# hsp-iit/online-detection

Measured on AMD Instinct MI355X. Metric: FALKON fit+infer samples/sec (N=1e6 D=1024 M=1e4), higher is better.
Workload: dtype f32-accurate K_nM (X Z' as a two-term f16 split on the f16 MFMA, f32 accumulate) stored as 24-bit fixed point (step 2^-24) + f64 solver (preconditioner: K_MM, T and T^-1 in f64; the products of the A factor, which only preconditions, at f32 accuracy on the f16 MFMA)

## Files before the change

online-detection_amd/csrc/api.cpp:

```cpp
#include "odx_common.h"
#include <string.h>

namespace odx {
static thread_local char g_error[512] = "";

void set_error(const char* fmt, ...) {
  va_list ap;
  va_start(ap, fmt);
  vsnprintf(g_error, sizeof(g_error), fmt, ap);
  va_end(ap);
}
}

extern "C" const char* odx_last_error_string(void) { return odx::g_error; }

#include "odx_internal.h"
namespace odx {
struct OptSpec {
  const char* name;
  int def, lo, hi;
};
constexpr int T_INVERSE_UNMERGED_DEFAULT = 2;
static const OptSpec g_opt_spec[OPT_COUNT] = {
    {"h2_tile", 0, 0, 256}, {"precond", 0, 0, 2}, {"chain_helpers", -1, -1, 1}, {"rls_force_nt_gram", 0, 0, 1},
    {"rls_force_inverse_solve", 0, 0, 1}, {"t_inverse_unmerged", T_INVERSE_UNMERGED_DEFAULT, 0, 2}, {"t_inverse_force_stop", 0, 0, 1 << 20}};
static int g_opt[OPT_COUNT] = {0, 0, -1, 0, 0, T_INVERSE_UNMERGED_DEFAULT, 0};
int lib_option(int which) { return g_opt[which]; }
static int opt_index(const char* name) {
  if (name)
    for (int i = 0; i < OPT_COUNT; ++i)
      if (strcmp(name, g_opt_spec[i].name) == 0) return i;
  return -1;
}
}

extern "C" int odx_set_option(const char* name, int value) {
  const int i = odx::opt_index(name);
  ODX_REQUIRE(i >= 0, "odx_set_option: unknown option '%s'", name ? name : "(null)");
  const odx::OptSpec& sp = odx::g_opt_spec[i];
  ODX_REQUIRE(value >= sp.lo && value <= sp.hi && (i != odx::OPT_H2_TILE || value == 0 || value == 128 || value == 256),
              "odx_set_option: %s = %d out of range", name, value);
  odx::g_opt[i] = value;
  return ODX_OK;
}

extern "C" int odx_get_option(const char* name, int* value) {
  const int i = odx::opt_index(name);
  ODX_REQUIRE(i >= 0 && value, "odx_get_option: unknown option '%s'", name ? name : "(null)");
  *value = odx::g_opt[i];
  return ODX_OK;
}

extern "C" int odx_option_default(const char* name, int* value) {
  const int i = odx::opt_index(name);
  ODX_REQUIRE(i >= 0 && value, "odx_option_default: unknown option '%s'", name ? name : "(null)");
  *value = odx::g_opt_spec[i].def;
  return ODX_OK;
}

extern "C" int odx_version(void) { return 100; }

extern "C" int odx_device_cus(void) {
  int dev = 0;
  if (hipGetDevice(&dev) != hipSuccess) {
    odx::set_error("odx_device_cus: no HIP device");
    return ODX_ERR_HIP;
  }
  int cus = 0;
  if (hipDeviceGetAttribute(&cus, hipDeviceAttributeMultiprocessorCount, dev) != hipSuccess) {
    odx::set_error("odx_device_cus: attribute query failed");
    return ODX_ERR_HIP;
  }
  return cus;
// ... 38 lines not shown
```

online-detection_amd/csrc/dense_f64.hip:

```cpp
#include "odx_internal.h"
#include <vector>

namespace odx {

typedef double f64x2 __attribute__((ext_vector_type(2)));
typedef double f64x4v __attribute__((ext_vector_type(4)));

constexpr int DB_NB = POTRF_NB;
constexpr int DB_LD = DB_NB + 1;
constexpr int DB_XLD = 33;
constexpr int DB_NT = 512;
constexpr int DB_PQ = 3072 / DB_NT;

__device__ __forceinline__ double readlane_f64(double v, int src) {
  const long long b = __double_as_longlong(v);
  const unsigned lo = (unsigned)__builtin_amdgcn_readlane((int)(b & 0xffffffffll), src);
  const unsigned hi = (unsigned)__builtin_amdgcn_readlane((int)(b >> 32), src);
  return __longlong_as_double((long long)(((unsigned long long)hi << 32) | lo));
}

__device__ __forceinline__ void chol32_wave(double* s, double* rd, int J, int jb, int32_t* info, int info_base,
                                            int lane) {
  const int l = lane & 31;
  double row[32];
// ... 577 lines not shown
  ODX_CHECK_LAUNCH("add_diag_f64");
  return ODX_OK;
}

int fill_f64(double* A, int64_t lda, int64_t rows, int64_t cols, double value, hipStream_t stream) {
  if (rows <= 0 || cols <= 0) return ODX_OK;
  ODX_REQUIRE(rows < 65536 * 32768ll, "fill_f64: too many rows");
  for (int64_t r0 = 0; r0 < rows; r0 += 65535) {
    const int64_t nr = rows - r0 < 65535 ? rows - r0 : 65535;
    hipLaunchKernelGGL(fill_f64_kernel, dim3((unsigned)ceil_div(cols, 256), (unsigned)nr), dim3(256), 0, stream,
                       A + r0 * lda, lda, nr, cols, value);
  }
  ODX_CHECK_LAUNCH("fill_f64");
  return ODX_OK;
}

__global__ __launch_bounds__(DB_NT) void trtri_diag_kernel(const double* __restrict__ L, int64_t ldl, int64_t M,
                                                          double* __restrict__ Dinv, int64_t zstrideA,
                                                          int64_t zstrideD) {
  __shared__ double s[DB_NB * DB_LD];
  L += (int64_t)blockIdx.y * zstrideA;
  Dinv += (int64_t)blockIdx.y * zstrideD;
  __shared__ double xi[32 * DB_XLD];
  const int64_t r0 = (int64_t)blockIdx.x * DB_NB;
  const int jb = (int)(M - r0 < DB_NB ? M - r0 : DB_NB);
  __shared__ double rd[32];
  lds_load_lower_128(s, L + r0 * ldl + r0, ldl, jb);
  lds_trinv_128<false>(s, xi, rd, nullptr);
  lds_store_dinv_128(s, Dinv + (int64_t)blockIdx.x * DB_NB * DB_NB, jb);
}

struct SideStream {
  hipStream_t stream = nullptr;
  hipEvent_t fork = nullptr, join = nullptr;
  int device = -1;
  bool owned = true;
};

static std::vector<uint32_t> g_side_mask;
static hipStream_t g_given_helper[2] = {nullptr, nullptr};

constexpr int64_t CHAIN_HELPER_MIN_M = 4096;

static bool chain_helpers(int64_t M) {
  const int o = lib_option(OPT_CHAIN_HELPERS);
  if (o == 0 || o == 1) return o == 1;
  return M >= CHAIN_HELPER_MIN_M;
}

struct SideEntry {
  int device;
  hipStream_t caller;
  SideStream ss[2];
};
static thread_local std::vector<SideEntry*> g_side_pool;

static int release_side_streams(bool wait = true) {
  for (SideEntry* e : g_side_pool) {
    for (SideStream& s : e->ss) {
      if (s.stream != nullptr) {
        if (wait) ODX_CHECK_HIP(hipStreamSynchronize(s.stream));
        if (s.owned) ODX_CHECK_HIP(hipStreamDestroy(s.stream));
      }
      if (s.fork != nullptr) ODX_CHECK_HIP(hipEventDestroy(s.fork));
      if (s.join != nullptr) ODX_CHECK_HIP(hipEventDestroy(s.join));
    }
    delete e;
  }
  g_side_pool.clear();
  return ODX_OK;
}

static int side_stream(SideStream** out, int slot, hipStream_t caller, int64_t M) {
  typedef SideEntry Entry;
  std::vector<Entry*>& pool = g_side_pool;
  int dev = 0;
  ODX_CHECK_HIP(hipGetDevice(&dev));
  ODX_REQUIRE(slot >= 0 && slot < 2, "side_stream: bad slot");
  if (!chain_helpers(M)) {
    static thread_local SideStream inl[2];
    SideStream& s = inl[slot];
    if (s.fork == nullptr || s.device != dev) {
      ODX_CHECK_HIP(hipEventCreateWithFlags(&s.fork, hipEventDisableTiming));
      ODX_CHECK_HIP(hipEventCreateWithFlags(&s.join, hipEventDisableTiming));
      s.device = dev;
    }
    s.stream = caller;
    *out = &s;
    return ODX_OK;
  }
  Entry* e = nullptr;
  for (Entry* c : pool)
    if (c->device == dev && c->caller == caller) e = c;
  if (e == nullptr) {
    e = new Entry();
    e->device = dev;
    e->caller = caller;
    pool.push_back(e);
  }
  SideStream& s = e->ss[slot];
  if (s.stream == nullptr) {
    s.owned = true;
    if (g_given_helper[slot] != nullptr && g_side_mask.empty()) {
      s.stream = g_given_helper[slot];
      s.owned = false;
    } else if (!g_side_mask.empty()) {
      ODX_CHECK_HIP(hipExtStreamCreateWithCUMask(&s.stream, (uint32_t)g_side_mask.size(), g_side_mask.data()));
    } else if (slot == 1) {
      int lo = 0, hi = 0;
      ODX_CHECK_HIP(hipDeviceGetStreamPriorityRange(&lo, &hi));
      ODX_CHECK_HIP(hipStreamCreateWithPriority(&s.stream, hipStreamNonBlocking, lo));
    } else {
      ODX_CHECK_HIP(hipStreamCreateWithFlags(&s.stream, hipStreamNonBlocking));
    }
    ODX_CHECK_HIP(hipEventCreateWithFlags(&s.fork, hipEventDisableTiming));
    ODX_CHECK_HIP(hipEventCreateWithFlags(&s.join, hipEventDisableTiming));
    s.device = dev;
  }
  *out = &s;
  return ODX_OK;
}

constexpr int POTRF_NBO = 512;

static bool precond_split(int64_t M) {
  const int o = lib_option(OPT_PRECOND);
  if (o == 1) return false;
  if (o == 2) return true;
  return M >= 4096;
}
static int64_t precond_pack_units(int64_t M) { return 2 * M * h2_f64_packed_ld(M); }
static int64_t precond_split_doubles(int64_t M) { return (precond_pack_units(M) + 2 * M * POTRF_NBO) / 2 + 2; }
static float split_scale_for(double bound) {
  int e = 0;
  frexp(bound > 1e-300 ? bound : 1.0, &e);
  return ldexpf(1.f, 12 - e);
}


int potrf_f64(double* A, int64_t lda, int64_t M, double* Dinv, int32_t* info, hipStream_t stream, const ZBatch& zb, uint32_t* pk,
              int64_t pk_buf, int64_t pk_z, float pk_scale) {
  constexpr int NB = POTRF_NB;
  ODX_REQUIRE(lda % 2 == 0 && aligned16(A) && aligned16(Dinv), "potrf_f64: A/Dinv must be 16-byte aligned, lda even");
  const int Z = zb.count;
  ODX_REQUIRE(Z >= 1 && Z <= ODX_MAX_ZBATCH && zb.strideA % 2 == 0 && zb.strideD % 2 == 0,
              "potrf_f64: class batch of 1..%d matrices, even strides", ODX_MAX_ZBATCH);
  auto zgemm = [&](GemmParams<double>& g) {
    g.zbatches = Z; g.zstrideA = zb.strideA; g.zstrideB = zb.strideA; g.zstrideC = zb.strideA;
  };
  ODX_CHECK_HIP(hipFuncSetAttribute(reinterpret_cast<const void*>(trsm128_kernel), hipFuncAttributeMaxDynamicSharedMemorySize,
                                    TS_LDS_BYTES));
  SideStream* look = nullptr;
  ODX_PROPAGATE(side_stream(&look, 1, stream, M));
  bool pending = false;
  for (int64_t K0 = 0; K0 < M; K0 += POTRF_NBO) {
    const int64_t kbo = M - K0 < POTRF_NBO ? M - K0 : POTRF_NBO;
    for (int64_t k0 = K0; k0 < K0 + kbo; k0 += NB) {
      const int jb = (int)(M - k0 < NB ? M - k0 : NB);
      double* D = Dinv + (k0 / NB) * NB * NB;
      hipLaunchKernelGGL((potrf_diag_kernel<NB, false>), dim3((unsigned)Z), dim3(DB_NT), 0, stream, A + k0 * lda + k0, lda,
                         jb, D, info, (int)k0, zb.strideA, zb.strideD);
      ODX_CHECK_LAUNCH("potrf_diag");
      const int64_t m = M - k0 - jb;
      if (m <= 0) break;
      double* A21 = A + (k0 + jb) * lda + k0;
      hipLaunchKernelGGL(trsm128_kernel, dim3((unsigned)ceil_div(m, TS_R), (unsigned)Z), dim3(256), TS_LDS_BYTES, stream,
                         A21, lda, m, A + k0 * lda + k0, D + NB * NB - 4096, zb.strideA, zb.strideD);
      ODX_CHECK_LAUNCH("trsm128");
      const int64_t pc = (K0 + kbo) - (k0 + jb);
      if (pc > 0) {
        GemmParams<double> u;
        u.A = A21; u.lda = lda; u.B = A21; u.ldb = lda; u.C = A + (k0 + jb) * lda + (k0 + jb); u.ldc = lda;
        u.m = m; u.n = pc; u.k = jb; u.alpha = -1.0; u.beta = 1.0; u.flags = ODX_GEMM_LOWER_ONLY;
        zgemm(u);
        ODX_PROPAGATE(launch_gemm_f64(u, stream));
      }
    }
    const int64_t mt = M - K0 - kbo;
    if (mt > 0) {
      double* P = A + (K0 + kbo) * lda + K0;
      const int64_t nw = mt < POTRF_NBO ? mt : POTRF_NBO;
      if (pending) {
        ODX_CHECK_HIP(hipStreamWaitEvent(stream, look->join, 0));
        pending = false;
      }
      const int64_t mr = mt - nw;
      double minus1[ODX_MAX_ZBATCH];
      for (int z = 0; z < Z; ++z) minus1[z] = -1.0;
      uint32_t* Pk = pk ? pk + ((K0 / POTRF_NBO) & 1) * pk_buf : nullptr;
      if (Pk) {
        ODX_PROPAGATE(split_f64(P, lda, zb.strideA, mt, kbo, pk_scale, Pk, POTRF_NBO, pk_z, Z, stream));
        ODX_PROPAGATE(gemm_h2_f64(Pk, POTRF_NBO, pk_z, pk_scale, Pk, POTRF_NBO, pk_z, pk_scale, A + (K0 + kbo) * (lda + 1), lda,
                                  zb.strideA, mt, nw, kbo, minus1, 1.0, ODX_GEMM_LOWER_ONLY, Z, stream));
      } else {
        GemmParams<double> u;
        u.A = P; u.lda = lda; u.B = P; u.ldb = lda; u.C = A + (K0 + kbo) * (lda + 1); u.ldc = lda;
        u.m = mt; u.n = nw; u.k = kbo; u.alpha = -1.0; u.beta = 1.0; u.flags = ODX_GEMM_LOWER_ONLY;
        zgemm(u);
        ODX_PROPAGATE(launch_gemm_f64(u, stream));
      }
      if (mr > 0) {
        ODX_CHECK_HIP(hipEventRecord(look->fork, stream));
        ODX_CHECK_HIP(hipStreamWaitEvent(look->stream, look->fork, 0));
        if (Pk) {
          ODX_PROPAGATE(gemm_h2_f64(Pk + nw * POTRF_NBO, POTRF_NBO, pk_z, pk_scale, Pk + nw * POTRF_NBO, POTRF_NBO, pk_z, pk_scale,
                                    A + (K0 + kbo + nw) * (lda + 1), lda, zb.strideA, mr, mr, kbo, minus1, 1.0, ODX_GEMM_LOWER_ONLY, Z,
                                    look->stream));
        } else {
          double* P2 = P + nw * lda;
          GemmParams<double> r;
          r.A = P2; r.lda = lda; r.B = P2; r.ldb = lda; r.C = A + (K0 + kbo + nw) * (lda + 1); r.ldc = lda;
// ... 346 lines not shown
  SideStream* side = nullptr;
  ODX_PROPAGATE(side_stream(&side, 0, s, M));
  hipStream_t s2 = side->stream;
  const int64_t wld = precond_ld(M), ldzd = precond_ldz(D);
  const int64_t dsz = ceil_div(M, POTRF_NB) * POTRF_NB * POTRF_NB;
  double* Zd = static_cast<double*>(workspace);
  double* zsq = Zd + M * ldzd;
  double* W0 = zsq + round_up(M, 2);
  double* W1 = W0 + M * wld;
  double* W2 = W1 + M * wld;
  double* W3 = W2 + M * wld;
  double* DinvT = W3 + M * wld;
  double* DinvA = DinvT + dsz;
  const bool split = precond_split(M);
  const int64_t ldpt = h2_f64_packed_ld(M);
  uint32_t* Tk = reinterpret_cast<uint32_t*>(DinvA + dsz);
  uint32_t* Pk = Tk + precond_pack_units(M);
  double* WA = L > 1 ? static_cast<double*>(workspace) + round_up(odx_falkon_precond_workspace_bytes(M, D), 16) / (int64_t)sizeof(double) : W2;

  ODX_CHECK_HIP(hipMemsetAsync(info, 0, (size_t)L * sizeof(int32_t), s));
  ODX_CHECK_HIP(hipMemsetAsync(Zd, 0, (size_t)(M * ldzd) * sizeof(double), s));
  ODX_PROPAGATE(odx_convert_f32_f64(Z, ldz, Zd, ldzd, M, D, stream));
  ODX_CHECK_HIP(hipMemsetAsync(W0, 0, (size_t)(M * wld) * sizeof(double), s));
  ODX_PROPAGATE(gauss_kmm_f64(Zd, ldzd, M, D, sigma, eps * (double)M, W0, wld, zsq, s, kind));
  ODX_PROPAGATE(potrf_f64(W0, wld, M, DinvT, info, s));
  for (int l = 1; l < L; ++l)
    ODX_CHECK_HIP(hipMemcpyAsync(info + l, info, sizeof(int32_t), hipMemcpyDeviceToDevice, s));
  ODX_CHECK_HIP(hipEventRecord(side->fork, s));
  ODX_CHECK_HIP(hipStreamWaitEvent(s2, side->fork, 0));
  ODX_PROPAGATE(fill_f64(LTi, ld, M, M, 0.0, s2));
  ODX_PROPAGATE(fill_f64(LTit, ld, M, M, 0.0, s2));
  ODX_PROPAGATE(trtri_from_diag_f64(W0, wld, M, DinvT, LTi, LTit, ld, W3, s2));
  ODX_CHECK_HIP(hipEventRecord(side->join, s2));
  ODX_CHECK_HIP(hipMemsetAsync(W1, 0, (size_t)(M * wld) * sizeof(double), s));
  ODX_PROPAGATE(transpose_f64(W0, wld, W1, wld, M, M, s));
  ODX_CHECK_HIP(hipMemsetAsync(W2, 0, (size_t)(M * wld) * sizeof(double), s));
  if (split) {
    const float st = split_scale_for(sqrt(1.0 + eps * 65536.0));
    const double a1 = 1.0 / (double)M;
    ODX_PROPAGATE(split_f64(W1, wld, 0, M, M, st, Tk, ldpt, 0, 1, s));
    ODX_PROPAGATE(gemm_h2_f64(Tk, ldpt, 0, st, Tk, ldpt, 0, st, W2, wld, 0, M, M, M, &a1, 0.0,
                              ODX_GEMM_LOWER_ONLY | ODX_GEMM_A_UPPER | ODX_GEMM_B_UPPER, 1, s));
  } else {
    GemmParams<double> g;
    g.A = W1; g.lda = wld; g.B = W1; g.ldb = wld; g.C = W2; g.ldc = wld;
    g.m = M; g.n = M; g.k = M; g.alpha = 1.0 / (double)M; g.beta = 0.0;
    g.flags = ODX_GEMM_LOWER_ONLY | ODX_GEMM_A_UPPER | ODX_GEMM_B_UPPER;
    ODX_PROPAGATE(launch_gemm_f64(g, s));
  }
  for (int l = 0; l < L; ++l) {
    const double lam = lams[l];
    if (WA != W2) ODX_CHECK_HIP(hipMemcpyAsync(WA, W2, (size_t)(M * wld) * sizeof(double), hipMemcpyDeviceToDevice, s));
    ODX_PROPAGATE(add_diag_f64(WA, wld, M, lam, s));
    if (split) ODX_PROPAGATE(potrf_f64(WA, wld, M, DinvA, info + l, s, ZBatch(), Pk, M * POTRF_NBO, 0, split_scale_for(sqrt(1.0 + eps + lam))));
    else ODX_PROPAGATE(potrf_f64(WA, wld, M, DinvA, info + l, s));
    if (l == 0) ODX_CHECK_HIP(hipStreamWaitEvent(s, side->join, 0));
    ODX_PROPAGATE(fill_f64(LAi[l], ld, M, M, 0.0, s));
    ODX_PROPAGATE(fill_f64(LAit[l], ld, M, M, 0.0, s));
    if (split && eps + lam > 0.0)
      ODX_PROPAGATE(trtri_from_diag_f64(WA, wld, M, DinvA, LAi[l], LAit[l], ld, W1, s, ZBatch(), Tk, precond_pack_units(M), 0,
                                        sqrt(1.0 + eps + lam), 1.0 / sqrt(eps + lam)));
    else
      ODX_PROPAGATE(trtri_from_diag_f64(WA, wld, M, DinvA, LAi[l], LAit[l], ld, W1, s));
  }
  return ODX_OK;
}

extern "C" int64_t odx_falkon_precond_batched_workspace_bytes(int64_t Mmax, int D, int B) {
  if (Mmax <= 0 || D <= 0 || B <= 0) return 0;
  const int64_t ld = precond_ld(Mmax), ldzd = precond_ldz(D);
  const int64_t per = Mmax * ldzd + round_up(Mmax, 2) + 4 * Mmax * ld + 2 * ceil_div(Mmax, POTRF_NB) * POTRF_NB * POTRF_NB +
                      precond_split_doubles(Mmax);
  return per * B * (int64_t)sizeof(double);
}

static int falkon_precond_batched_f64_impl(const float* const* Z, const int64_t* ldz, const int64_t* M, int B,
                                           int64_t Mmax, int D, double sigma, double lam, double eps, int64_t t_stop, double* out,
                                           int64_t ld, int64_t out_stride, int32_t* info, void* workspace,
                                           int64_t workspace_bytes, odx_stream_t stream);

extern "C" int odx_falkon_precond_batched_f64(const float* const* Z, const int64_t* ldz, const int64_t* M, int B,
                                              int64_t Mmax, int D, double sigma, double lam, double eps, double* out,
                                              int64_t ld, int64_t out_stride, int32_t* info, void* workspace,
                                              int64_t workspace_bytes, odx_stream_t stream) {
  const int rc = falkon_precond_batched_f64_impl(Z, ldz, M, B, Mmax, D, sigma, lam, eps, 0, out, ld, out_stride, info, workspace, workspace_bytes, stream);
  return rc;
}
// ... 14 lines not shown
  ODX_REQUIRE(Z && ldz && M && out && info && workspace && Mmax > 0 && D > 0 && sigma > 0,
              "odx_falkon_precond_batched_f64: null pointer or bad size");
  ODX_REQUIRE(ld % 2 == 0 && ld >= Mmax && aligned16(out) && out_stride % 2 == 0 && out_stride >= 4 * Mmax * ld,
              "odx_falkon_precond_batched_f64: out must be 16-byte aligned, ld even >= Mmax, out_stride >= 4 Mmax ld");
  ODX_REQUIRE(aligned16(workspace), "odx_falkon_precond_batched_f64: workspace must be 16-byte aligned");
  for (int b = 0; b < B; ++b)
    ODX_REQUIRE(Z[b] && M[b] > 0 && M[b] <= Mmax, "odx_falkon_precond_batched_f64: class %d: need 0 < M <= Mmax", b);
  if (workspace_bytes < odx_falkon_precond_batched_workspace_bytes(Mmax, D, B)) {
    set_error("odx_falkon_precond_batched_f64: workspace too small");
    return ODX_ERR_WORKSPACE;
  }
  hipStream_t s = as_stream(stream);
  SideStream* side = nullptr;
  ODX_PROPAGATE(side_stream(&side, 0, s, Mmax));
  hipStream_t s2 = side->stream;
  const int64_t wld = precond_ld(Mmax), ldzd = precond_ldz(D);
  const int64_t dsz = ceil_div(Mmax, POTRF_NB) * POTRF_NB * POTRF_NB;
  const int64_t zper = Mmax * ldzd + round_up(Mmax, 2), wsz = Mmax * wld;
  double* Zd0 = static_cast<double*>(workspace);
  double* W0 = Zd0 + (int64_t)B * zper;
  double* W1 = W0 + (int64_t)B * wsz;
  double* W2 = W1 + (int64_t)B * wsz;
  double* W3 = W2 + (int64_t)B * wsz;
  double* DinvT = W3 + (int64_t)B * wsz;
  double* DinvA = DinvT + (int64_t)B * dsz;
  double* LTi = out, *LTit = out + Mmax * ld, *LAi = out + 2 * Mmax * ld, *LAit = out + 3 * Mmax * ld;
  const bool split = precond_split(Mmax);
  const int64_t ldpt = h2_f64_packed_ld(Mmax);
  uint32_t* Tk = reinterpret_cast<uint32_t*>(DinvA + (int64_t)B * dsz);
  uint32_t* Pk = Tk + (int64_t)B * precond_pack_units(Mmax);

  ODX_CHECK_HIP(hipMemsetAsync(info, 0, (size_t)B * sizeof(int32_t), s));
  ODX_CHECK_HIP(hipMemsetAsync(Zd0, 0, (size_t)((int64_t)B * zper) * sizeof(double), s));
  ODX_CHECK_HIP(hipMemsetAsync(W0, 0, (size_t)(3 * (int64_t)B * wsz) * sizeof(double), s));
  if (out_stride == 4 * Mmax * ld) {
    ODX_CHECK_HIP(hipMemsetAsync(out, 0, (size_t)((int64_t)B * out_stride) * sizeof(double), s));
  } else {
    for (int b = 0; b < B; ++b)
      ODX_CHECK_HIP(hipMemsetAsync(out + (int64_t)b * out_stride, 0, (size_t)(4 * Mmax * ld) * sizeof(double), s));
  }
  VecBatch kb;
  kb.B = B;
  for (int b = 0; b < B; ++b) {
    ODX_PROPAGATE(odx_convert_f32_f64(Z[b], ldz[b], Zd0 + (int64_t)b * zper, ldzd, M[b], D, stream));
    kb.M[b] = (int)M[b];
    kb.scale[b] = eps * (double)M[b];
  }
  ODX_PROPAGATE(gauss_kmm_f64_batched(Zd0, ldzd, zper, Mmax * ldzd, kb, D, sigma, W0, wld, wsz, s));
  for (int b = 0; b < B; ++b)
    if (M[b] < Mmax) ODX_PROPAGATE(add_diag_f64(W0 + (int64_t)b * wsz + M[b] * (wld + 1), wld, Mmax - M[b], 1.0, s));
  ZBatch zt;
  zt.count = B; zt.strideA = wsz; zt.strideD = dsz; zt.strideO = out_stride; zt.strideW = wsz;
  ODX_PROPAGATE(potrf_f64(W0, wld, Mmax, DinvT, info, s, zt));
  ODX_CHECK_HIP(hipEventRecord(side->fork, s));
  ODX_CHECK_HIP(hipStreamWaitEvent(s2, side->fork, 0));
  ODX_PROPAGATE(trtri_from_diag_f64(W0, wld, Mmax, DinvT, LTi, LTit, ld, W3, s2, zt, nullptr, 0, 0, 1.0, 1.0, t_stop));
  ODX_CHECK_HIP(hipEventRecord(side->join, s2));
  ODX_PROPAGATE(transpose_f64(W0, wld, W1, wld, Mmax, Mmax, s, B, wsz, wsz));
  if (split) {
    const float st = split_scale_for(sqrt(1.0 + eps * 65536.0)), sa = split_scale_for(sqrt(1.0 + eps + lam));
    double a1[ODX_MAX_ZBATCH];
    for (int b = 0; b < B; ++b) a1[b] = 1.0 / (double)M[b];
    ODX_PROPAGATE(split_f64(W1, wld, wsz, Mmax, Mmax, st, Tk, ldpt, precond_pack_units(Mmax), B, s));
    ODX_PROPAGATE(gemm_h2_f64(Tk, ldpt, precond_pack_units(Mmax), st, Tk, ldpt, precond_pack_units(Mmax), st, W2, wld, wsz, Mmax, Mmax, Mmax, a1, 0.0,
                              ODX_GEMM_LOWER_ONLY | ODX_GEMM_A_UPPER | ODX_GEMM_B_UPPER, B, s));
    ODX_PROPAGATE(add_diag_f64(W2, wld, Mmax, lam, s, B, wsz));
    ODX_PROPAGATE(potrf_f64(W2, wld, Mmax, DinvA, info, s, zt, Pk, (int64_t)B * Mmax * POTRF_NBO, Mmax * POTRF_NBO, sa));
  } else {
    GemmParams<double> g;
    g.A = W1; g.lda = wld; g.B = W1; g.ldb = wld; g.C = W2; g.ldc = wld;
    g.m = Mmax; g.n = Mmax; g.k = Mmax; g.beta = 0.0;
    g.flags = ODX_GEMM_LOWER_ONLY | ODX_GEMM_A_UPPER | ODX_GEMM_B_UPPER;
    g.zbatches = B; g.zstrideA = wsz; g.zstrideB = wsz; g.zstrideC = wsz;
    g.zalpha_on = 1;
    for (int b = 0; b < B; ++b) g.zalpha[b] = 1.0 / (double)M[b];
    ODX_PROPAGATE(launch_gemm_f64(g, s));
    ODX_PROPAGATE(add_diag_f64(W2, wld, Mmax, lam, s, B, wsz));
    ODX_PROPAGATE(potrf_f64(W2, wld, Mmax, DinvA, info, s, zt));
  }
  ODX_CHECK_HIP(hipStreamWaitEvent(s, side->join, 0));
  if (split && eps + lam > 0.0)
    return trtri_from_diag_f64(W2, wld, Mmax, DinvA, LAi, LAit, ld, W1, s, zt, Tk, precond_pack_units(Mmax), precond_pack_units(Mmax),
                               sqrt(1.0 + eps + lam), 1.0 / sqrt(eps + lam));
  return trtri_from_diag_f64(W2, wld, Mmax, DinvA, LAi, LAit, ld, W1, s, zt);
}

extern "C" int odx_set_side_stream_cu_mask(const uint32_t* mask, int words) {
  ODX_REQUIRE(words >= 0 && words <= 64 && (words == 0 || mask != nullptr), "odx_set_side_stream_cu_mask: bad argument");
  g_side_mask.assign(mask, mask + words);
  return ODX_OK;
}

extern "C" int odx_set_helper_streams(odx_stream_t s0, odx_stream_t s1) {
  g_given_helper[0] = reinterpret_cast<hipStream_t>(s0);
  g_given_helper[1] = reinterpret_cast<hipStream_t>(s1);
  return ODX_OK;
}

extern "C" int odx_release_helper_streams(void) {
  return odx::release_side_streams(false);
// ... 2 lines not shown
```

online-detection_amd/csrc/gauss_h2.hip:

```cpp
#include <stdlib.h>
#include <type_traits>
#include "gemm_core.h"
#include "odx_internal.h"

namespace odx {

typedef _Float16 f16x8 __attribute__((ext_vector_type(8)));

constexpr int H2_KT = 64;

__global__ __launch_bounds__(256) void absmax_f32_kernel(const float* __restrict__ X, int64_t ldx, int64_t n, int D,
                                                         unsigned int* __restrict__ out) {
  unsigned int m = 0;
  const int lane = threadIdx.x & 63;
  for (int64_t r = (int64_t)blockIdx.x * 4 + (threadIdx.x >> 6); r < n; r += (int64_t)gridDim.x * 4) {
    const float* x = X + r * ldx;
    for (int c0 = lane * 4; c0 < D; c0 += 1024) {
      u32x4 v[4];
#pragma unroll
      for (int u = 0; u < 4; ++u) {
        const int c = c0 + 256 * u;
        v[u] = (c < D) ? *reinterpret_cast<const u32x4*>(x + c) : u32x4{0u, 0u, 0u, 0u};
      }
#pragma unroll
// ... 1486 lines not shown
  *reinterpret_cast<u32x4*>(P + row * ldp + f) = v;
}

__global__ __launch_bounds__(256) void split_f64_kernel(const double* __restrict__ X, int64_t ldx, int64_t zsx, int64_t rows, int cols,
                                                        float s, uint32_t* __restrict__ P, int64_t ldp, int64_t zsp) {
  const int groups = (int)((cols + H2_KT - 1) / H2_KT) * 8;
  const int64_t row = blockIdx.y;
  const int g = blockIdx.x * 256 + threadIdx.x;
  if (g >= groups || row >= rows) return;
  const double* x = X + (int64_t)blockIdx.z * zsx + row * ldx + (int64_t)g * 8;
  double v[8];
  if (g * 8 + 8 <= cols) {
#pragma unroll
    for (int q = 0; q < 8; q += 2) {
      const f64x2 a = *reinterpret_cast<const f64x2*>(x + q);
      v[q] = a[0];
      v[q + 1] = a[1];
    }
  } else {
#pragma unroll
    for (int q = 0; q < 8; ++q) v[q] = (g * 8 + q < cols) ? x[q] : 0.0;
  }
  f16x8 hi, lo;
#pragma unroll
  for (int q = 0; q < 8; ++q) {
    const float t = (float)(v[q] * (double)s);
    const _Float16 h = (_Float16)t;
    hi[q] = h;
    lo[q] = (_Float16)(t - (float)h);
  }
  uint32_t* dst = P + (int64_t)blockIdx.z * zsp + row * ldp + (int64_t)(g >> 2) * 32 + (g & 3) * 4;
  *reinterpret_cast<f16x8*>(dst) = hi;
  *reinterpret_cast<f16x8*>(dst + 16) = lo;
}

struct H2F64Params {
  const uint32_t* PA; int64_t ldpa, zsa, bsa;
  const uint32_t* PB; int64_t ldpb, zsb, bsb;
  double* C; int64_t ldc, zsc, bsc;
  double* C2; int64_t ldc2, zsc2, bsc2;
  int64_t m, n, k;
  int64_t rg_total, rg_off, rg_step;
  int k_is_m;
  int flags;
  double beta;
  double alpha[ODX_MAX_ZBATCH];
};

struct SplitBlocks {
  const double* X; int64_t ldx, bsx, zsx;
  uint32_t* P; int64_t ldp, bsp, zsp;
  int64_t rows, cols;
  int64_t rg_total, rg_off, rg_step;
  int rows_ragged, cols_ragged, Z;
  float s;
};

__global__ __launch_bounds__(256) void split_f64_blocks_kernel(SplitBlocks p) {
  const int b = blockIdx.z / p.Z, z = blockIdx.z % p.Z;
  int64_t rg = p.rg_total - p.rg_off - (int64_t)b * p.rg_step;
  const int64_t rows = p.rows_ragged ? (rg < p.rows ? (rg > 0 ? rg : 0) : p.rows) : p.rows;
  const int64_t cols = p.cols_ragged ? (rg < p.cols ? (rg > 0 ? rg : 0) : p.cols) : p.cols;
  const int64_t row = blockIdx.y;
  const int groups = (int)((cols + H2_KT - 1) / H2_KT) * 8;
  const int g = blockIdx.x * 256 + threadIdx.x;
  if (g >= groups || row >= rows) return;
// ... 332 lines not shown

static int check_packed_pair(const char* who, int64_t dp, int64_t ldpx, int64_t ldpz, const void* PX, const void* PZ) {
  ODX_REQUIRE(ldpx % 4 == 0 && ldpz % 4 == 0 && ldpx >= dp && ldpz >= dp && aligned16(PX) && aligned16(PZ),
              "%s: packed operands must be 16-byte aligned with ld %% 4 == 0 and ld >= %lld 4-byte units", who, (long long)dp);
  ODX_REQUIRE(ldpx < (1 << 24) && ldpz < (1 << 24), "%s: leading dimensions must stay below 2^24 (32-bit tile offsets)", who);
  return ODX_OK;
}

static int check_knm_block(const char* who, int fmt, int64_t M, const void* K, int64_t ldk, const void* Klo, int64_t ldlo) {
  const int64_t ldmin = odx_knm_ld(M, fmt);
  ODX_REQUIRE(K && ldk >= ldmin && ldk % (fmt == ODX_KNM_F32 ? 4 : 8) == 0 && aligned16(K),
              "%s: K must be 16-byte aligned with ldk a multiple of %d and >= %lld", who, fmt == ODX_KNM_F32 ? 4 : 8, (long long)ldmin);
  if (fmt == ODX_KNM_U24)
    ODX_REQUIRE(Klo && ldlo >= ldmin && ldlo % 8 == 0 && aligned16(Klo), "%s: the low-byte plane must be 16-byte aligned with ldlo %% 8 == 0, ldlo >= roundup(M, 8)", who);
  ODX_REQUIRE(ldk < (1 << 24), "%s: leading dimensions must stay below 2^24 (32-bit tile offsets)", who);
  return ODX_OK;
}

int64_t h2_f64_packed_ld(int64_t cols) { return round_up(cols, H2_KT); }

int split_f64(const double* X, int64_t ldx, int64_t zsx, int64_t rows, int64_t cols, float scale, uint32_t* P, int64_t ldp,
              int64_t zsp, int z, hipStream_t stream) {
  if (rows <= 0 || cols <= 0 || z <= 0) return ODX_OK;
  ODX_REQUIRE(ldx % 2 == 0 && aligned16(X) && zsx % 2 == 0, "split_f64: X must be 16-byte aligned with even ld / class stride");
  ODX_REQUIRE(ldp % 4 == 0 && ldp >= round_up(cols, H2_KT) && aligned16(P) && zsp % 4 == 0, "split_f64: packed rows cover roundup(cols, 64)");
  ODX_REQUIRE(rows < 65536 && z < 65536, "split_f64: too many rows");
  const int groups = (int)(round_up(cols, H2_KT) / 8);
  hipLaunchKernelGGL(split_f64_kernel, dim3((unsigned)ceil_div(groups, 256), (unsigned)rows, (unsigned)z), dim3(256), 0, stream, X, ldx, zsx,
                     rows, (int)cols, scale, P, ldp, zsp);
  ODX_CHECK_LAUNCH("split_f64");
  return ODX_OK;
}

int split_f64_blocks(const SplitBlocksArgs& a, hipStream_t stream) {
  if (a.rows <= 0 || a.cols <= 0 || a.nb <= 0 || a.Z <= 0) return ODX_OK;
  ODX_REQUIRE(a.ldx % 2 == 0 && aligned16(a.X) && a.zsx % 2 == 0 && a.bsx % 2 == 0, "split_f64_blocks: X blocks must be 16-byte aligned");
  ODX_REQUIRE(a.ldp % 4 == 0 && a.ldp >= round_up(a.cols, H2_KT) && aligned16(a.P) && a.zsp % 4 == 0 && a.bsp % 4 == 0,
              "split_f64_blocks: packed rows cover roundup(cols, 64)");
  ODX_REQUIRE(a.rows < 65536 && (int64_t)a.nb * a.Z < 65536, "split_f64_blocks: too many rows / blocks");
  SplitBlocks p;
  p.X = a.X; p.ldx = a.ldx; p.bsx = a.bsx; p.zsx = a.zsx; p.P = a.P; p.ldp = a.ldp; p.bsp = a.bsp; p.zsp = a.zsp;
  p.rows = a.rows; p.cols = a.cols; p.rg_total = a.rg_total; p.rg_off = a.rg_off; p.rg_step = a.rg_step;
  p.rows_ragged = a.rows_ragged; p.cols_ragged = a.cols_ragged; p.Z = a.Z; p.s = a.scale;
  const int groups = (int)(round_up(a.cols, H2_KT) / 8);
  hipLaunchKernelGGL(split_f64_blocks_kernel, dim3((unsigned)ceil_div(groups, 256), (unsigned)a.rows, (unsigned)(a.nb * a.Z)), dim3(256), 0,
                     stream, p);
  ODX_CHECK_LAUNCH("split_f64_blocks");
  return ODX_OK;
}

int gemm_h2_f64_ex(const H2F64Args& a, hipStream_t stream) {
  if (a.m <= 0 || a.n <= 0 || a.zcount <= 0 || a.nb <= 0) return ODX_OK;
  ODX_REQUIRE(a.zcount <= ODX_MAX_ZBATCH && a.nb < 65536 && a.ldc % 2 == 0 && a.zsc % 2 == 0 && a.bsc % 2 == 0 && aligned16(a.C),
              "gemm_h2_f64: C must be 16-byte aligned, even ld / strides");
  ODX_REQUIRE(a.C2 == nullptr || (a.ldc2 % 2 == 0 && a.zsc2 % 2 == 0 && a.bsc2 % 2 == 0 && aligned16(a.C2)), "gemm_h2_f64: C2 alignment");
  ODX_REQUIRE(!(a.flags & ODX_GEMM_STORE_T) || a.beta == 0.0, "gemm_h2_f64: a transposed store cannot accumulate");
  ODX_REQUIRE(a.ldpa < (1 << 24) && a.ldpb < (1 << 24) && a.ldpa >= round_up(a.k, H2_KT) && a.ldpb >= round_up(a.k, H2_KT),
              "gemm_h2_f64: packed leading dimensions");
  H2F64Params p;
  p.PA = a.PA; p.ldpa = a.ldpa; p.zsa = a.zsa; p.bsa = a.bsa; p.PB = a.PB; p.ldpb = a.ldpb; p.zsb = a.zsb; p.bsb = a.bsb;
  p.C = a.C; p.ldc = a.ldc; p.zsc = a.zsc; p.bsc = a.bsc; p.C2 = a.C2; p.ldc2 = a.ldc2; p.zsc2 = a.zsc2; p.bsc2 = a.bsc2;
  p.m = a.m; p.n = a.n; p.k = a.k; p.rg_total = a.rg_total; p.rg_off = a.rg_off; p.rg_step = a.rg_step; p.k_is_m = a.k_is_m;
  p.flags = a.flags; p.beta = a.beta;
  for (int z = 0; z < a.zcount; ++z) p.alpha[z] = a.alpha[z] / ((double)a.sa * (double)a.sb);
  const int64_t wt = round_up(ceil_div(a.m, W_BM), 4) * ceil_div(a.n, W_BN);
  ODX_REQUIRE(wt < (1ll << 31), "gemm_h2_f64: grid too large");
// ... 1153 lines not shown
```

online-detection_amd/csrc/odx_internal.h:

```cpp
#pragma once
#include "odx_common.h"

namespace odx {
enum LibOpt {
  OPT_H2_TILE = 0,
  OPT_PRECOND,
  OPT_CHAIN_HELPERS,
  OPT_RLS_FORCE_NT_GRAM,
  OPT_RLS_FORCE_INVERSE_SOLVE,
  OPT_T_INVERSE_UNMERGED,
  OPT_T_INVERSE_FORCE_STOP,
  OPT_COUNT
};
int lib_option(int which);


constexpr int ODX_MAX_ZBATCH = 32;

template <typename T>
struct GemmParams {
  const T* A = nullptr; int64_t lda = 0;
  const T* B = nullptr; int64_t ldb = 0;
  T* C = nullptr; int64_t ldc = 0;
  T* C2 = nullptr; int64_t ldc2 = 0;
  int64_t m = 0, n = 0, k = 0;
  T alpha = T(1), beta = T(0);
  int flags = 0;
  int batches = 1;
  int64_t strideA = 0, strideB = 0, strideC = 0, strideC2 = 0;
  int64_t ragged_total = 0, ragged_off = 0, ragged_step = 0;
  int ragged_k_is_m = 0;
  int vec_epilogue = 0;
  int zbatches = 1;
  int64_t zstrideA = 0, zstrideB = 0, zstrideC = 0, zstrideC2 = 0;
  int zalpha_on = 0;
  T zalpha[ODX_MAX_ZBATCH] = {};
  int zk_on = 0;
  int64_t zkoff[ODX_MAX_ZBATCH] = {};
  int64_t zklen[ODX_MAX_ZBATCH] = {};
};

int launch_gemm_f64(const GemmParams<double>& p, hipStream_t stream);
int launch_gemm_f32(const GemmParams<float>& p, hipStream_t stream);

// ... 28 lines not shown
int knm_passq_batched(int B, const void* const* Khi, const int64_t* ldk, const void* const* Klo, const int64_t* ldlo, int fmt,
                      const int64_t* n, const int64_t* M, const double* v, int64_t vstride, double* out, int64_t ostride,
                      void* workspace, int64_t workspace_bytes, hipStream_t stream);

int pass_cus();
int check_q_block(const char* who, const void* K, int64_t ldk, const void* Klo, int64_t ldlo, int fmt, int64_t M);

bool knm_pass_batch_cfg(int B, const int64_t* M, int* nt, int* ch, int* r);
int64_t knm_pass_batched_workspace_bytes(int B, const int64_t* n, const int64_t* M);
int knm_pass_batched(int B, const float* const* K, const int64_t* ldk, const int64_t* n, const int64_t* M, const double* v,
                     int64_t vstride, double* out, int64_t ostride, void* workspace, int64_t workspace_bytes,
                     hipStream_t stream);

struct VecBatch {
  int B = 1;
  int M[ODX_MAX_ZBATCH] = {};
  double scale[ODX_MAX_ZBATCH] = {};
};
int trmv_batched_f64(const double* Tri, int64_t ld, int64_t tri_stride, int uplo, const VecBatch& vb, const double* x,
                     int64_t xstride, bool scaled, double beta, const double* z, int64_t zstride, double* y,
                     int64_t ystride, hipStream_t stream);
int cg_init_batched(const VecBatch& vb, const double* Bv, double* X, double* R, double* P, double* state, int64_t vstride,
                    hipStream_t stream);
int cg_step_batched(const VecBatch& vb, double* X, double* R, const double* P, const double* AP, double* state,
                    double cg_eps, int full_grad, int64_t vstride, hipStream_t stream);
int cg_finish_batched(const VecBatch& vb, const double* R, double* P, double* state, double cg_eps, double tol,
                      int64_t vstride, hipStream_t stream);
int cg_full_residual_batched(const VecBatch& vb, const double* Bv, const double* AX, double* R, int64_t vstride,
                             hipStream_t stream);

int64_t h2_f64_packed_ld(int64_t cols);
int split_f64(const double* X, int64_t ldx, int64_t zsx, int64_t rows, int64_t cols, float scale, uint32_t* P, int64_t ldp,
              int64_t zsp, int z, hipStream_t stream);
struct SplitBlocksArgs {
  const double* X = nullptr; int64_t ldx = 0, bsx = 0, zsx = 0;
  uint32_t* P = nullptr; int64_t ldp = 0, bsp = 0, zsp = 0;
  int64_t rows = 0, cols = 0;
  int64_t rg_total = 0, rg_off = 0, rg_step = 0;
  int rows_ragged = 0, cols_ragged = 0, nb = 1, Z = 1;
  float scale = 1.f;
};
int split_f64_blocks(const SplitBlocksArgs& a, hipStream_t stream);
struct H2F64Args {
  const uint32_t* PA = nullptr; int64_t ldpa = 0, zsa = 0, bsa = 0; float sa = 1.f;
  const uint32_t* PB = nullptr; int64_t ldpb = 0, zsb = 0, bsb = 0; float sb = 1.f;
  double* C = nullptr; int64_t ldc = 0, zsc = 0, bsc = 0;
  double* C2 = nullptr; int64_t ldc2 = 0, zsc2 = 0, bsc2 = 0;
  int64_t m = 0, n = 0, k = 0;
  int64_t rg_total = 0, rg_off = 0, rg_step = 0;
  int k_is_m = 0, flags = 0, zcount = 1, nb = 1;
  double beta = 0.0;
  double alpha[ODX_MAX_ZBATCH] = {};
};
int gemm_h2_f64_ex(const H2F64Args& a, hipStream_t stream);
int gemm_h2_f64(const uint32_t* PA, int64_t ldpa, int64_t zsa, float sa, const uint32_t* PB, int64_t ldpb, int64_t zsb, float sb,
                double* C, int64_t ldc, int64_t zsc, int64_t m, int64_t n, int64_t k, const double* alpha, double beta, int flags,
                int zcount, hipStream_t stream);

int gauss_kmm_f64(const double* Zd, int64_t ldz, int64_t M, int D, double sigma, double diag_add, double* Kmm,
                  int64_t ldk, double* zsq , hipStream_t stream, int kind = ODX_KERNEL_GAUSS);

int gauss_kmm_f64_batched(const double* Zd, int64_t ldz, int64_t z_stride, int64_t zsq_off, const VecBatch& vb, int D,
                          double sigma, double* Kmm, int64_t ldk, int64_t k_stride, hipStream_t stream, int kind = ODX_KERNEL_GAUSS);

}
```

online-detection_amd/odx/plan.py:

```python
from dataclasses import dataclass, field

HBM_BYTES_MI355X = 288e9
BUDGET_FRACTION = 0.9
MAX_CHAIN_CLASSES = 6
RESERVE_BYTES = 3e9


def _round_up(x, m):
    return (int(x) + m - 1) // m * m


STREAM_BYTES = 256 << 20


def knm_format_rule(n, M, storage="auto", wide_tile=True):
    if storage in ("f32", "u24", "bf16", "stream"):
        return storage
    if n * M >= (1 << 27) and M >= 1024 and wide_tile:
        return "u24"
    return "f32"


def knm_bytes_rule(n, M, fmt):
    if fmt == "stream":
        return STREAM_BYTES
    if fmt == "f32":
        return int(n) * _round_up(M, 4) * 4
    return int(n) * _round_up(M, 8) * (3 if fmt == "u24" else 2)


def chain_workspace_bytes(M, D):
    ld = _round_up(M, 2)
    split = (2 * M * _round_up(M, 64) + 2 * M * 512) // 2 + 2
    ldz = _round_up(D, 2)
    ldz += 64 if ldz % 128 == 0 else 0
    return (M * ldz + ld + 4 * M * ld + 2 * ((M + 127) // 128) * 128 * 128 + split) * 8


def factor_bytes(M):
    return 4 * M * _round_up(M, 2) * 8


def divisors_desc(world):
    return [b for b in range(world, 0, -1) if world % b == 0]


def owners_of_batch(k, size, world, b):
    R = world // b
    base = (k % R) * b
    return [base + j for j in range(size)]


def lockstep_batches(classes, world, b):
    classes = list(classes)
    return [(classes[k0:k0 + b], owners_of_batch(k0 // b, len(classes[k0:k0 + b]), world, b)) for k0 in range(0, len(classes), b)]


def precond_groups(n_units, G):
    groups, g0 = [], 0
    for size in (1, 2, 3):
        if g0 < n_units and size < G:
            groups.append(list(range(g0, min(g0 + size, n_units))))
            g0 += size
    while g0 < n_units:
        groups.append(list(range(g0, min(g0 + G, n_units))))
        g0 += G
# ... 78 lines not shown
```

Before: 195,300.

## Batch Cholesky trailing updates over several panels and fuse transpose into split packing

The blocked Cholesky on the split-f16 path now defers the trailing-matrix update. Panels are packed into a wider buffer holding up to four panels, and the full trailing GEMM runs once per group with a deeper K instead of once per panel. The intermediate panels only update the region inside the current group, and the lookahead side stream now uses an extra 'mid' event for ordering. Separately, a new kernel packs the transposed lower factor straight into the f16 split format, which skips the f64 transpose and its workspace memset. Both changes raise GEMM efficiency and cut memory traffic in the preconditioner, at the cost of larger pack workspace and more complex stream synchronisation.

```diff
diff --git a/online-detection_amd/csrc/api.cpp b/online-detection_amd/csrc/api.cpp
--- a/online-detection_amd/csrc/api.cpp
+++ b/online-detection_amd/csrc/api.cpp
@@ -21,10 +21,12 @@
   int def, lo, hi;
 };
 constexpr int T_INVERSE_UNMERGED_DEFAULT = 2;
+constexpr int CHOL_UPDATE_PANELS_DEFAULT = 4;
 static const OptSpec g_opt_spec[OPT_COUNT] = {
     {"h2_tile", 0, 0, 256}, {"precond", 0, 0, 2}, {"chain_helpers", -1, -1, 1}, {"rls_force_nt_gram", 0, 0, 1},
-    {"rls_force_inverse_solve", 0, 0, 1}, {"t_inverse_unmerged", T_INVERSE_UNMERGED_DEFAULT, 0, 2}, {"t_inverse_force_stop", 0, 0, 1 << 20}};
-static int g_opt[OPT_COUNT] = {0, 0, -1, 0, 0, T_INVERSE_UNMERGED_DEFAULT, 0};
+    {"rls_force_inverse_solve", 0, 0, 1}, {"t_inverse_unmerged", T_INVERSE_UNMERGED_DEFAULT, 0, 2}, {"t_inverse_force_stop", 0, 0, 1 << 20},
+    {"chol_update_panels", CHOL_UPDATE_PANELS_DEFAULT, 1, 4}, {"precond_pack_transpose", 0, 0, 1}};
+static int g_opt[OPT_COUNT] = {0, 0, -1, 0, 0, T_INVERSE_UNMERGED_DEFAULT, 0, CHOL_UPDATE_PANELS_DEFAULT, 0};
 int lib_option(int which) { return g_opt[which]; }
 static int opt_index(const char* name) {
   if (name)
@@ -38,7 +40,8 @@
   const int i = odx::opt_index(name);
   ODX_REQUIRE(i >= 0, "odx_set_option: unknown option '%s'", name ? name : "(null)");
   const odx::OptSpec& sp = odx::g_opt_spec[i];
-  ODX_REQUIRE(value >= sp.lo && value <= sp.hi && (i != odx::OPT_H2_TILE || value == 0 || value == 128 || value == 256),
+  ODX_REQUIRE(value >= sp.lo && value <= sp.hi && (i != odx::OPT_H2_TILE || value == 0 || value == 128 || value == 256) &&
+                  (i != odx::OPT_CHOL_UPDATE_PANELS || value != 3),
               "odx_set_option: %s = %d out of range", name, value);
   odx::g_opt[i] = value;
   return ODX_OK;
diff --git a/online-detection_amd/csrc/dense_f64.hip b/online-detection_amd/csrc/dense_f64.hip
--- a/online-detection_amd/csrc/dense_f64.hip
+++ b/online-detection_amd/csrc/dense_f64.hip
@@ -633,7 +633,7 @@
 
 struct SideStream {
   hipStream_t stream = nullptr;
-  hipEvent_t fork = nullptr, join = nullptr;
+  hipEvent_t fork = nullptr, join = nullptr, mid = nullptr;
   int device = -1;
   bool owned = true;
 };
@@ -665,6 +665,7 @@
       }
       if (s.fork != nullptr) ODX_CHECK_HIP(hipEventDestroy(s.fork));
       if (s.join != nullptr) ODX_CHECK_HIP(hipEventDestroy(s.join));
+      if (s.mid != nullptr) ODX_CHECK_HIP(hipEventDestroy(s.mid));
     }
     delete e;
   }
@@ -684,6 +685,7 @@
     if (s.fork == nullptr || s.device != dev) {
       ODX_CHECK_HIP(hipEventCreateWithFlags(&s.fork, hipEventDisableTiming));
       ODX_CHECK_HIP(hipEventCreateWithFlags(&s.join, hipEventDisableTiming));
+      ODX_CHECK_HIP(hipEventCreateWithFlags(&s.mid, hipEventDisableTiming));
       s.device = dev;
     }
     s.stream = caller;
@@ -716,6 +718,7 @@
     }
     ODX_CHECK_HIP(hipEventCreateWithFlags(&s.fork, hipEventDisableTiming));
     ODX_CHECK_HIP(hipEventCreateWithFlags(&s.join, hipEventDisableTiming));
+    ODX_CHECK_HIP(hipEventCreateWithFlags(&s.mid, hipEventDisableTiming));
     s.device = dev;
   }
   *out = &s;
@@ -731,7 +734,9 @@
   return M >= 4096;
 }
 static int64_t precond_pack_units(int64_t M) { return 2 * M * h2_f64_packed_ld(M); }
-static int64_t precond_split_doubles(int64_t M) { return (precond_pack_units(M) + 2 * M * POTRF_NBO) / 2 + 2; }
+static int chol_update_panels() { return lib_option(OPT_CHOL_UPDATE_PANELS); }
+static int64_t precond_panel_units(int64_t M) { return M * POTRF_NBO * chol_update_panels(); }
+static int64_t precond_split_doubles(int64_t M) { return (precond_pack_units(M) + 2 * precond_panel_units(M)) / 2 + 2; }
 static float split_scale_for(double bound) {
   int e = 0;
   frexp(bound > 1e-300 ? bound : 1.0, &e);
@@ -754,6 +759,8 @@
   SideStream* look = nullptr;
   ODX_PROPAGATE(side_stream(&look, 1, stream, M));
   bool pending = false;
+  bool mid_pending = false;
+  const int S = pk ? chol_update_panels() : 1;
   for (int64_t K0 = 0; K0 < M; K0 += POTRF_NBO) {
     const int64_t kbo = M - K0 < POTRF_NBO ? M - K0 : POTRF_NBO;
     for (int64_t k0 = K0; k0 < K0 + kbo; k0 += NB) {
@@ -778,6 +785,53 @@
       }
     }
     const int64_t mt = M - K0 - kbo;
+    if (S > 1) {
+      if (mt <= 0) continue;
+      const int64_t W = (int64_t)S * POTRF_NBO, sp = K0 / W, q = (K0 / POTRF_NBO) % S;
+      const int64_t SPend = (sp + 1) * W;
+      const int64_t c0 = K0 + kbo;
+      uint32_t* Pb = pk + (sp & 1) * pk_buf;
+      uint32_t* Pq = Pb + q * POTRF_NBO * W + q * POTRF_NBO;
+      double minus1[ODX_MAX_ZBATCH];
+      for (int z = 0; z < Z; ++z) minus1[z] = -1.0;
+      ODX_PROPAGATE(split_f64(A + c0 * lda + K0, lda, zb.strideA, mt, kbo, pk_scale, Pq, W, pk_z, Z, stream));
+      if (q < S - 1) {
+        if (mid_pending) {
+          ODX_CHECK_HIP(hipStreamWaitEvent(stream, look->mid, 0));
+          mid_pending = false;
+        }
+        const int64_t n = (SPend < M ? SPend : M) - c0;
+        ODX_PROPAGATE(gemm_h2_f64(Pq, W, pk_z, pk_scale, Pq, W, pk_z, pk_scale, A + c0 * (lda + 1), lda, zb.strideA, mt, n, kbo, minus1, 1.0,
+                                  ODX_GEMM_LOWER_ONLY, Z, stream));
+        continue;
+      }
+      uint32_t* Pr = Pb + (int64_t)(S - 1) * POTRF_NBO * W;
+      const int64_t nw = mt < POTRF_NBO ? mt : POTRF_NBO;
+      if (pending) {
+        ODX_CHECK_HIP(hipStreamWaitEvent(stream, look->join, 0));
+        pending = false;
+      }
+      mid_pending = false;
+      ODX_PROPAGATE(gemm_h2_f64(Pr, W, pk_z, pk_scale, Pr, W, pk_z, pk_scale, A + c0 * (lda + 1), lda, zb.strideA, mt, nw, W, minus1, 1.0,
+                                ODX_GEMM_LOWER_ONLY, Z, stream));
+      const int64_t mr = mt - nw;
+      if (mr > 0) {
+        const int64_t n1 = mr < W - POTRF_NBO ? mr : W - POTRF_NBO, mr2 = mr - n1;
+        ODX_CHECK_HIP(hipEventRecord(look->fork, stream));
+        ODX_CHECK_HIP(hipStreamWaitEvent(look->stream, look->fork, 0));
+        ODX_PROPAGATE(gemm_h2_f64(Pr + nw * W, W, pk_z, pk_scale, Pr + nw * W, W, pk_z, pk_scale, A + (c0 + nw) * (lda + 1), lda, zb.strideA,
+                                  mr, n1, W, minus1, 1.0, ODX_GEMM_LOWER_ONLY, Z, look->stream));
+        ODX_CHECK_HIP(hipEventRecord(look->mid, look->stream));
+        mid_pending = true;
+        if (mr2 > 0)
+          ODX_PROPAGATE(gemm_h2_f64(Pr + (nw + n1) * W, W, pk_z, pk_scale, Pr + (nw + n1) * W, W, pk_z, pk_scale,
+                                    A + (c0 + nw + n1) * (lda + 1), lda, zb.strideA, mr2, mr2, W, minus1, 1.0, ODX_GEMM_LOWER_ONLY, Z,
+                                    look->stream));
+        ODX_CHECK_HIP(hipEventRecord(look->join, look->stream));
+        pending = true;
+      }
+      continue;
+    }
     if (mt > 0) {
       double* P = A + (K0 + kbo) * lda + K0;
       const int64_t nw = mt < POTRF_NBO ? mt : POTRF_NBO;
@@ -1190,13 +1244,17 @@
   ODX_PROPAGATE(fill_f64(LTit, ld, M, M, 0.0, s2));
   ODX_PROPAGATE(trtri_from_diag_f64(W0, wld, M, DinvT, LTi, LTit, ld, W3, s2));
   ODX_CHECK_HIP(hipEventRecord(side->join, s2));
-  ODX_CHECK_HIP(hipMemsetAsync(W1, 0, (size_t)(M * wld) * sizeof(double), s));
-  ODX_PROPAGATE(transpose_f64(W0, wld, W1, wld, M, M, s));
+  const bool t_f64 = !split || lib_option(OPT_PRECOND_PACK_TRANSPOSE) != 0;
+  if (t_f64) {
+    ODX_CHECK_HIP(hipMemsetAsync(W1, 0, (size_t)(M * wld) * sizeof(double), s));
+    ODX_PROPAGATE(transpose_f64(W0, wld, W1, wld, M, M, s));
+  }
   ODX_CHECK_HIP(hipMemsetAsync(W2, 0, (size_t)(M * wld) * sizeof(double), s));
   if (split) {
     const float st = split_scale_for(sqrt(1.0 + eps * 65536.0));
     const double a1 = 1.0 / (double)M;
-    ODX_PROPAGATE(split_f64(W1, wld, 0, M, M, st, Tk, ldpt, 0, 1, s));
+    if (t_f64) ODX_PROPAGATE(split_f64(W1, wld, 0, M, M, st, Tk, ldpt, 0, 1, s));
+    else ODX_PROPAGATE(split_f64_lower_t(W0, wld, 0, M, st, Tk, ldpt, 0, 1, s));
     ODX_PROPAGATE(gemm_h2_f64(Tk, ldpt, 0, st, Tk, ldpt, 0, st, W2, wld, 0, M, M, M, &a1, 0.0,
                               ODX_GEMM_LOWER_ONLY | ODX_GEMM_A_UPPER | ODX_GEMM_B_UPPER, 1, s));
   } else {
@@ -1210,7 +1268,7 @@
     const double lam = lams[l];
     if (WA != W2) ODX_CHECK_HIP(hipMemcpyAsync(WA, W2, (size_t)(M * wld) * sizeof(double), hipMemcpyDeviceToDevice, s));
     ODX_PROPAGATE(add_diag_f64(WA, wld, M, lam, s));
-    if (split) ODX_PROPAGATE(potrf_f64(WA, wld, M, DinvA, info + l, s, ZBatch(), Pk, M * POTRF_NBO, 0, split_scale_for(sqrt(1.0 + eps + lam))));
+    if (split) ODX_PROPAGATE(potrf_f64(WA, wld, M, DinvA, info + l, s, ZBatch(), Pk, precond_panel_units(M), 0, split_scale_for(sqrt(1.0 + eps + lam))));
     else ODX_PROPAGATE(potrf_f64(WA, wld, M, DinvA, info + l, s));
     if (l == 0) ODX_CHECK_HIP(hipStreamWaitEvent(s, side->join, 0));
     ODX_PROPAGATE(fill_f64(LAi[l], ld, M, M, 0.0, s));
@@ -1291,7 +1349,13 @@
 
   ODX_CHECK_HIP(hipMemsetAsync(info, 0, (size_t)B * sizeof(int32_t), s));
   ODX_CHECK_HIP(hipMemsetAsync(Zd0, 0, (size_t)((int64_t)B * zper) * sizeof(double), s));
-  ODX_CHECK_HIP(hipMemsetAsync(W0, 0, (size_t)(3 * (int64_t)B * wsz) * sizeof(double), s));
+  const bool t_f64 = !split || lib_option(OPT_PRECOND_PACK_TRANSPOSE) != 0;
+  if (t_f64) {
+    ODX_CHECK_HIP(hipMemsetAsync(W0, 0, (size_t)(3 * (int64_t)B * wsz) * sizeof(double), s));
+  } else {
+    ODX_CHECK_HIP(hipMemsetAsync(W0, 0, (size_t)((int64_t)B * wsz) * sizeof(double), s));
+    ODX_CHECK_HIP(hipMemsetAsync(W2, 0, (size_t)((int64_t)B * wsz) * sizeof(double), s));
+  }
   if (out_stride == 4 * Mmax * ld) {
     ODX_CHECK_HIP(hipMemsetAsync(out, 0, (size_t)((int64_t)B * out_stride) * sizeof(double), s));
   } else {
@@ -1315,16 +1379,17 @@
   ODX_CHECK_HIP(hipStreamWaitEvent(s2, side->fork, 0));
   ODX_PROPAGATE(trtri_from_diag_f64(W0, wld, Mmax, DinvT, LTi, LTit, ld, W3, s2, zt, nullptr, 0, 0, 1.0, 1.0, t_stop));
   ODX_CHECK_HIP(hipEventRecord(side->join, s2));
-  ODX_PROPAGATE(transpose_f64(W0, wld, W1, wld, Mmax, Mmax, s, B, wsz, wsz));
+  if (t_f64) ODX_PROPAGATE(transpose_f64(W0, wld, W1, wld, Mmax, Mmax, s, B, wsz, wsz));
   if (split) {
     const float st = split_scale_for(sqrt(1.0 + eps * 65536.0)), sa = split_scale_for(sqrt(1.0 + eps + lam));
     double a1[ODX_MAX_ZBATCH];
     for (int b = 0; b < B; ++b) a1[b] = 1.0 / (double)M[b];
-    ODX_PROPAGATE(split_f64(W1, wld, wsz, Mmax, Mmax, st, Tk, ldpt, precond_pack_units(Mmax), B, s));
+    if (t_f64) ODX_PROPAGATE(split_f64(W1, wld, wsz, Mmax, Mmax, st, Tk, ldpt, precond_pack_units(Mmax), B, s));
+    else ODX_PROPAGATE(split_f64_lower_t(W0, wld, wsz, Mmax, st, Tk, ldpt, precond_pack_units(Mmax), B, s));
     ODX_PROPAGATE(gemm_h2_f64(Tk, ldpt, precond_pack_units(Mmax), st, Tk, ldpt, precond_pack_units(Mmax), st, W2, wld, wsz, Mmax, Mmax, Mmax, a1, 0.0,
                               ODX_GEMM_LOWER_ONLY | ODX_GEMM_A_UPPER | ODX_GEMM_B_UPPER, B, s));
     ODX_PROPAGATE(add_diag_f64(W2, wld, Mmax, lam, s, B, wsz));
-    ODX_PROPAGATE(potrf_f64(W2, wld, Mmax, DinvA, info, s, zt, Pk, (int64_t)B * Mmax * POTRF_NBO, Mmax * POTRF_NBO, sa));
+    ODX_PROPAGATE(potrf_f64(W2, wld, Mmax, DinvA, info, s, zt, Pk, (int64_t)B * precond_panel_units(Mmax), precond_panel_units(Mmax), sa));
   } else {
     GemmParams<double> g;
     g.A = W1; g.lda = wld; g.B = W1; g.ldb = wld; g.C = W2; g.ldc = wld;
diff --git a/online-detection_amd/csrc/gauss_h2.hip b/online-detection_amd/csrc/gauss_h2.hip
--- a/online-detection_amd/csrc/gauss_h2.hip
+++ b/online-detection_amd/csrc/gauss_h2.hip
@@ -1542,6 +1542,53 @@
   uint32_t* dst = P + (int64_t)blockIdx.z * zsp + row * ldp + (int64_t)(g >> 2) * 32 + (g & 3) * 4;
   *reinterpret_cast<f16x8*>(dst) = hi;
   *reinterpret_cast<f16x8*>(dst + 16) = lo;
+}
+
+__global__ __launch_bounds__(256) void split_f64_lower_t_kernel(const double* __restrict__ L, int64_t ldl, int64_t zsl, int64_t M, float s,
+                                                                uint32_t* __restrict__ P, int64_t ldp, int64_t zsp) {
+  __shared__ double tile[64][65];
+  const int64_t r0 = (int64_t)blockIdx.y * 64, c0 = (int64_t)blockIdx.x * 64;
+  const int tid = threadIdx.x;
+  const bool any = c0 + 63 >= r0;
+  if (any) {
+    L += (int64_t)blockIdx.z * zsl;
+    f64x2 v[8];
+#pragma unroll
+    for (int q = 0; q < 8; ++q) {
+      const int e = tid + 256 * q, ci = e >> 5, rj = (e & 31) * 2;
+      const bool ok = c0 + ci < M && r0 + rj < M && r0 + rj <= c0 + ci;
+      v[q] = ok ? *reinterpret_cast<const f64x2*>(L + (c0 + ci) * ldl + r0 + rj) : f64x2{0.0, 0.0};
+    }
+#pragma unroll
+    for (int q = 0; q < 8; ++q) {
+      const int e = tid + 256 * q, ci = e >> 5, rj = (e & 31) * 2;
+      const int64_t c = c0 + ci, r = r0 + rj;
+      tile[ci][rj] = (c < M && r <= c) ? v[q][0] : 0.0;
+      tile[ci][rj + 1] = (c < M && r + 1 <= c) ? v[q][1] : 0.0;
+    }
+    __syncthreads();
+  }
+  P += (int64_t)blockIdx.z * zsp;
+#pragma unroll
+  for (int pass = 0; pass < 2; ++pass) {
+    const int g = tid & 7, rr = pass * 32 + (tid >> 3);
+    if (r0 + rr >= M) continue;
+    double v[8];
+#pragma unroll
+    for (int q = 0; q < 8; ++q) v[q] = any ? tile[8 * g + q][rr] : 0.0;
+    f16x8 hi, lo;
+#pragma unroll
+    for (int q = 0; q < 8; ++q) {
+      const double xs = v[q] * (double)s;
+      const float t = (float)xs;
+      const _Float16 h = (_Float16)xs;
+      hi[q] = h;
+      lo[q] = (_Float16)(t - (float)h);
+    }
+    uint32_t* dst = P + (r0 + rr) * ldp + c0 + (int64_t)(g >> 2) * 32 + (g & 3) * 4;
+    *reinterpret_cast<f16x8*>(dst) = hi;
+    *reinterpret_cast<f16x8*>(dst + 16) = lo;
+  }
 }
 
 struct H2F64Params {
@@ -1940,6 +1987,19 @@
   return ODX_OK;
 }
 
+int split_f64_lower_t(const double* L, int64_t ldl, int64_t zsl, int64_t M, float scale, uint32_t* P, int64_t ldp, int64_t zsp, int z,
+                      hipStream_t stream) {
+  if (M <= 0 || z <= 0) return ODX_OK;
+  ODX_REQUIRE(ldl % 2 == 0 && ldl >= M && aligned16(L) && zsl % 2 == 0, "split_f64_lower_t: L must be 16-byte aligned with even ld >= M / class stride");
+  ODX_REQUIRE(ldp % 4 == 0 && ldp >= round_up(M, H2_KT) && aligned16(P) && zsp % 4 == 0, "split_f64_lower_t: packed rows cover roundup(M, 64)");
+  ODX_REQUIRE(M < 65536 * 64 && z < 65536, "split_f64_lower_t: too many rows");
+  const int64_t tiles = ceil_div(M, H2_KT);
+  hipLaunchKernelGGL(split_f64_lower_t_kernel, dim3((unsigned)tiles, (unsigned)tiles, (unsigned)z), dim3(256), 0, stream, L, ldl, zsl, M,
+                     scale, P, ldp, zsp);
+  ODX_CHECK_LAUNCH("split_f64_lower_t");
+  return ODX_OK;
+}
+
 int split_f64_blocks(const SplitBlocksArgs& a, hipStream_t stream) {
   if (a.rows <= 0 || a.cols <= 0 || a.nb <= 0 || a.Z <= 0) return ODX_OK;
   ODX_REQUIRE(a.ldx % 2 == 0 && aligned16(a.X) && a.zsx % 2 == 0 && a.bsx % 2 == 0, "split_f64_blocks: X blocks must be 16-byte aligned");
diff --git a/online-detection_amd/csrc/odx_internal.h b/online-detection_amd/csrc/odx_internal.h
--- a/online-detection_amd/csrc/odx_internal.h
+++ b/online-detection_amd/csrc/odx_internal.h
@@ -10,6 +10,8 @@
   OPT_RLS_FORCE_INVERSE_SOLVE,
   OPT_T_INVERSE_UNMERGED,
   OPT_T_INVERSE_FORCE_STOP,
+  OPT_CHOL_UPDATE_PANELS,
+  OPT_PRECOND_PACK_TRANSPOSE,
   OPT_COUNT
 };
 int lib_option(int which);
@@ -104,6 +106,8 @@
 int64_t h2_f64_packed_ld(int64_t cols);
 int split_f64(const double* X, int64_t ldx, int64_t zsx, int64_t rows, int64_t cols, float scale, uint32_t* P, int64_t ldp,
               int64_t zsp, int z, hipStream_t stream);
+int split_f64_lower_t(const double* L, int64_t ldl, int64_t zsl, int64_t M, float scale, uint32_t* P, int64_t ldp, int64_t zsp, int z,
+                      hipStream_t stream);
 struct SplitBlocksArgs {
   const double* X = nullptr; int64_t ldx = 0, bsx = 0, zsx = 0;
   uint32_t* P = nullptr; int64_t ldp = 0, bsp = 0, zsp = 0;
diff --git a/online-detection_amd/odx/plan.py b/online-detection_amd/odx/plan.py
--- a/online-detection_amd/odx/plan.py
+++ b/online-detection_amd/odx/plan.py
@@ -29,9 +29,12 @@
     return int(n) * _round_up(M, 8) * (3 if fmt == "u24" else 2)
 
 
+CHOL_UPDATE_PANELS = 4
+
+
 def chain_workspace_bytes(M, D):
     ld = _round_up(M, 2)
-    split = (2 * M * _round_up(M, 64) + 2 * M * 512) // 2 + 2
+    split = (2 * M * _round_up(M, 64) + 2 * M * 512 * CHOL_UPDATE_PANELS) // 2 + 2
     ldz = _round_up(D, 2)
     ldz += 64 if ldz % 128 == 0 else 0
     return (M * ldz + ld + 4 * M * ld + 2 * ((M + 127) // 128) * 128 * 128 + split) * 8
```

After: 196,700 (median of 6 runs). About the same (+0.7%).
